# paulmillr/noble-bls12-381

Measured on AMD Instinct MI355X. Metric: pairings/sec, higher is better.
Workload: dtype int64; 1 GPU; batch of 4096 independent BLS12-381 pairings per GPU (Miller loop + final exponentiation, inputs pre-validated, bit-exact vs reference), inputs/outputs resident in HBM; batch_per_gpu=4096, batches_in_flight=12

## Files before the change

### include/nbls.h

```cpp
#ifndef NBLS_H
#define NBLS_H
#include <stddef.h>
#include <stdint.h>
#ifdef __cplusplus
extern "C" {
#endif

typedef struct nbls_ctx nbls_ctx;

#define NBLS_OK 0
#define NBLS_EINVAL (-1)
#define NBLS_EHIP (-2)
#define NBLS_ENOSUP (-3)
#define NBLS_ENOGPU (-4)
#define NBLS_EDECODE (-5)

int nbls_init(int device_id, nbls_ctx** out);
void nbls_destroy(nbls_ctx* ctx);
const char* nbls_strerror(int code);
int nbls_last_hip_error(nbls_ctx* ctx);

int nbls_pairing_batch(nbls_ctx* ctx, size_t n, const uint8_t* g1_aff, const uint8_t* g2_aff, int with_final_exp, int validate,
                       uint8_t* out_fp12, int8_t* status);
int nbls_pairing_batch_dev(nbls_ctx* ctx, size_t n, const void* d_g1_aff, const void* d_g2_aff, int with_final_exp,
// ... 193 lines not shown
                                            uint8_t* out_proofs48 , int8_t* status );
int  nbls_kzg_recover_cells_and_proofs_fk20(nbls_ctx* ctx, const nbls_kzg_fk20* fk, size_t n, const uint32_t* cell_offsets, const uint32_t* cell_index, const uint8_t* cells,
                                            uint8_t* out_cells, uint8_t* out_proofs48 , int8_t* status );

#define NBLS_ST_G16_C 30
typedef struct nbls_groth16_vk nbls_groth16_vk;
int  nbls_groth16_vk_create(nbls_ctx* ctx, size_t m, const uint8_t* alpha_g1_48, const uint8_t* beta_g2_96, const uint8_t* gamma_g2_96, const uint8_t* delta_g2_96,
                            const uint8_t* ic48 , int8_t* status , nbls_groth16_vk** out);
void nbls_groth16_vk_destroy(nbls_groth16_vk* vk);
int  nbls_groth16_vk_inputs(const nbls_groth16_vk* vk, size_t* m);
int  nbls_groth16_verify(nbls_ctx* ctx, const nbls_groth16_vk* vk, size_t n, const uint8_t* proofs192, const uint8_t* inputs32 , const uint8_t* seed32 ,
                         int* all_ok, int8_t* status );
int  nbls_groth16_prepare_inputs(nbls_ctx* ctx, const nbls_groth16_vk* vk, size_t n, const uint8_t* inputs32, uint8_t* out48 , int8_t* status );
int  nbls_groth16_input_sums(nbls_ctx* ctx, size_t n, size_t m, const uint8_t* inputs32, const uint8_t* weights32 , const int8_t* pre ,
                             uint8_t* out32 , int8_t* status );

#define NBLS_ST_G16_UNSATISFIED 24
typedef struct {
  unsigned log2_n; size_t n_vars, n_public , n_constraints ;
  const uint32_t *a_rows, *a_cols; const uint8_t* a_vals32;
  const uint32_t *b_rows, *b_cols; const uint8_t* b_vals32;
  const uint32_t *c_rows, *c_cols; const uint8_t* c_vals32;
  const uint8_t *alpha_g1_48, *beta_g1_48, *beta_g2_96, *delta_g1_48, *delta_g2_96;
  const uint8_t *a_query48 , *b_g1_query48 , *b_g2_query96 , *l_query48 , *h_query48 ;
} nbls_groth16_pk_desc;
typedef struct nbls_groth16_pk nbls_groth16_pk;
int  nbls_groth16_pk_create(nbls_ctx* ctx, const nbls_groth16_pk_desc* desc, int8_t* status , nbls_groth16_pk** out);
void nbls_groth16_pk_destroy(nbls_groth16_pk* pk);
int  nbls_groth16_pk_params(const nbls_groth16_pk* pk, unsigned* log2_n, size_t* n_vars, size_t* n_public);
int  nbls_groth16_pk_wiped(nbls_ctx* ctx, nbls_groth16_pk* pk, int* wiped);
int  nbls_groth16_prove(nbls_ctx* ctx, nbls_groth16_pk* pk, size_t n, const uint8_t* witness32 ,
                        const uint8_t* rs32 , uint8_t* out_proofs192, int8_t* status );
int  nbls_groth16_quotient(nbls_ctx* ctx, unsigned log2_n, size_t n, const uint8_t* a32, const uint8_t* b32, const uint8_t* c32 ,
                           uint8_t* out_h32 , int8_t* status );

int nbls_verify_batch_partial_dev(nbls_ctx* ctx, size_t n, const void* d_sig96 , const void* d_uniform256, const void* d_pk48,
                                  void* d_out_fp12, int* zero_flag, int8_t* pk_status , void* stream);

int nbls_miller_product_partial(nbls_ctx* ctx, size_t n, const uint8_t* g1_aff, const uint8_t* g2_aff, int validate, void** d_partial, int8_t* status);
int nbls_verify_batch_partial(nbls_ctx* ctx, size_t n, const uint8_t* sig96 , const uint8_t* msgs, const uint32_t* offsets, const uint8_t* pk48,
                              const uint8_t* dst, size_t dst_len, void** d_partial, int* zero_flag, int8_t* pk_status );
int nbls_miller_product_partial_into(nbls_ctx* ctx, size_t n, const uint8_t* g1_aff, const uint8_t* g2_aff, int validate, void* d_dst576, int8_t* status);
int nbls_verify_batch_partial_into(nbls_ctx* ctx, size_t n, const uint8_t* sig96 , const uint8_t* msgs, const uint32_t* offsets, const uint8_t* pk48,
                                   const uint8_t* dst, size_t dst_len, void* d_dst576, int* zero_flag, int8_t* pk_status );
const char* nbls_config_describe(void);
#define NBLS_ABI_VERSION 5
int nbls_abi_version(void);
int nbls_context_device(nbls_ctx* ctx);

int nbls_hw_queues(int* set_by_library);
typedef struct nbls_pool nbls_pool;
int nbls_pool_init(int device_id, int depth , nbls_pool** out);
#define NBLS_POOL_SPREAD_PRIORITIES 1u
int nbls_pool_init_ex(int device_id, int depth , unsigned flags, nbls_pool** out);
int nbls_pool_stream_priority(nbls_pool* p, int i, int* priority);
void nbls_pool_destroy(nbls_pool* p);
int nbls_pool_depth(const nbls_pool* p);
nbls_ctx* nbls_pool_context(nbls_pool* p, int i);
int nbls_pool_next_slot(nbls_pool* p);
int nbls_pool_pairing_batch_dev(nbls_pool* p, size_t n, const void* d_g1, const void* d_g2, int with_final_exp, void* d_out, int* slot);
int nbls_pool_synchronize(nbls_pool* p);

typedef struct nbls_multi nbls_multi;
int nbls_init_multi(int n_devices, const int* device_ids, nbls_multi** out);
void nbls_destroy_multi(nbls_multi* m);
int nbls_multi_device_count(const nbls_multi* m);
nbls_ctx* nbls_multi_context(nbls_multi* m, int i);
int nbls_multi_peer_access(const nbls_multi* m, int i);
int nbls_multi_pairing_batch(nbls_multi* m, size_t n, const uint8_t* g1_aff, const uint8_t* g2_aff, int with_final_exp, int validate,
                             uint8_t* out_fp12, int8_t* status);
int nbls_multi_miller_product(nbls_multi* m, size_t n, const uint8_t* g1_aff, const uint8_t* g2_aff, int final_exp, int validate,
                              uint8_t* out_fp12, int8_t* status);
int nbls_multi_verify_batch(nbls_multi* m, size_t n, const uint8_t* sig96, const uint8_t* msgs, const uint32_t* offsets, const uint8_t* pk48,
                            const uint8_t* dst, size_t dst_len, int* ok);

int nbls_program_stats(nbls_ctx* ctx, int prog, uint32_t* out8);
int nbls_device_synchronize(nbls_ctx* ctx);
int nbls_placement_probe(nbls_ctx* ctx, size_t n, uint64_t* out_blocks);
int nbls_field_kernel_raw(nbls_ctx* ctx, int kind, int form, size_t n, const uint8_t* in_raw, uint8_t* out_raw);
#define NBLS_N_PROGRAMS 128
#define NBLS_TUNE_SPLIT_MILLER_MIN 1
#define NBLS_TUNE_HALVES_MIN 2
#define NBLS_TUNE_EXPC_MIN 3
#define NBLS_TUNE_CHAIN_MAX 4
#define NBLS_TUNE_VERIFY_CHUNKS 5
#define NBLS_TUNE_VERIFY_LAST_PCT 6
#define NBLS_TUNE_VERIFY_PIPE_MIN 7
#define NBLS_TUNE_SAC_MAX 8
#define NBLS_TUNE_PT_LS2_MAX 9
#define NBLS_TUNE_WIDE_MAX 10
#define NBLS_TUNE_H2C_NORM_MIN 11
#define NBLS_TUNE_INV_WIDE_MAX 12
#define NBLS_TUNE_LS_MAX 13
#define NBLS_TUNE_LS2_MAX 14
#define NBLS_TUNE_POLY_SLAB 15
#define NBLS_TUNE_MSMB_WINDOW 16
#define NBLS_TUNE_MSMB_BIG 17
#define NBLS_TUNE_MSMB_SLAB 18
#define NBLS_TUNE_CELLS_CHUNK 20
#define NBLS_TUNE_G16_CHUNK 22
#define NBLS_TUNE_FE_TAIL_CHAIN 24
#define NBLS_TUNE_NTT_TAIL_BITS 26
#define NBLS_TUNE_NTT_PASS_BITS 27
#define NBLS_TUNE_FE_HEAD_CHAIN 29
#define NBLS_TUNE_INV_PRIO 30
#define NBLS_TUNE_G16P_ROW_WAVE 31
int nbls_set_tuning(nbls_ctx* ctx, int key, long long value);
int nbls_program_count(void);
// ... 14 lines not shown
```

### noble-bls12-381_amd/csrc/nbls_internal.h

```cpp
#pragma once
#include <hip/hip_runtime.h>
#include "config.h"
#include <cstdio>
#include <cstring>
#include <mutex>
#include <vector>
#include <initializer_list>
#include <new>
#include "nbls.h"
#include "programs.h"
#include "consts_gen.h"
#include "fp_inv.h"
#include "pow_exec.h"
#include "sha256.h"
#include "curve.h"
#include "bufs.h"
#include "verifier_frame.h"
#include <thread>

#include "launchers.h"
#include "wide_exec.h"
#include "aot.h"
#include <map>
#include <tuple>
// ... 189 lines not shown
    if (ctx->ev_last && ctx->ev_last_set && ctx->last_stream != s) hipStreamWaitEvent(s, ctx->ev_last, 0);
  }
  ~StreamOrder() { if (ctx->ev_last && hipEventRecord(ctx->ev_last, s) == hipSuccess) { ctx->ev_last_set = true; ctx->last_stream = s; } }
};

struct ForkGuard {
  bool armed = true; void* keys = nullptr; size_t key_bytes = 0;
  ~ForkGuard() { if (armed) { (void)hipDeviceSynchronize(); if (keys) (void)hipMemset(keys, 0, key_bytes); } }
};
struct Window {
  size_t first = 0;
  int half = 0;
  bool beside = false;
};
struct HostIO {
  nbls_ctx* ctx; std::vector<size_t> mine; hipStream_t s = nullptr; std::vector<std::pair<void*, size_t>> secrets; bool wiped = false;
  ~HostIO() {
    if (!mine.empty()) (void)hipStreamSynchronize(s ? s : ctx->stream);
    if (!wiped) for (auto& k : secrets) (void)hipMemset(k.first, 0, k.second);
    for (size_t i : mine) ctx->io_pool[i].busy = false;
  }
  void secret(void* p, size_t n) { if (p && n) secrets.push_back({p, n}); }
  int wipe(hipStream_t st) { for (auto& k : secrets) if (hipMemsetAsync(k.first, 0, k.second, st) != hipSuccess) return NBLS_EHIP; wiped = true; return NBLS_OK; }
  void* alloc(size_t n) {
    if (!n) n = 1;
    auto& pool = ctx->io_pool;
    size_t best = (size_t)-1;
    for (size_t i = 0; i < pool.size(); i++)
      if (!pool[i].busy && pool[i].p && pool[i].cap >= n && pool[i].cap / 4 <= n && (best == (size_t)-1 || pool[i].cap < pool[best].cap)) best = i;
    if (best != (size_t)-1) { pool[best].busy = true; mine.push_back(best); return pool[best].p; }
    static const size_t cap_bytes = (size_t)env_long("NBLS_IO_POOL_MB", 1024) << 20;
    const size_t cap = n + n / 8 + 256;
    for (size_t i = 0; i < pool.size() && ctx->io_pool_bytes + cap > cap_bytes; i++)
      if (!pool[i].busy && pool[i].p) { hipFree(pool[i].p); ctx->io_pool_bytes -= pool[i].cap; pool[i].p = nullptr; pool[i].cap = 0; }
    void* p = nullptr;
    if (hipMalloc(&p, cap) != hipSuccess) { (void)hipGetLastError(); return nullptr; }
    ctx->io_pool_bytes += cap;
    size_t slot = (size_t)-1;
    for (size_t i = 0; i < pool.size(); i++) if (!pool[i].p) { slot = i; break; }
    if (slot == (size_t)-1) { pool.push_back({nullptr, 0, false}); slot = pool.size() - 1; }
    pool[slot] = {p, cap, true};
    mine.push_back(slot);
    return p;
  }
};
#define LOCKED(ctx) std::lock_guard<std::recursive_mutex> g_((ctx)->mu); HIPCHK(hipSetDevice((ctx)->device)); hipStream_t s = (ctx)->stream; StreamOrder order_((ctx), s)
static inline hipStream_t call_stream(nbls_ctx* ctx, void* stream) { return stream ? (hipStream_t)stream : ctx->stream; }
#define DEV_ENTER(ctx, stream) std::lock_guard<std::recursive_mutex> g_((ctx)->mu); HIPCHK(hipSetDevice((ctx)->device)); hipStream_t s = call_stream((ctx), (stream)); StreamOrder order_((ctx), s)
#define WHOLE_CALL(ctx) std::lock_guard<std::recursive_mutex> whole_call_((ctx) ? (ctx)->mu : g_null_mu)

struct VerifyIn;
int nbls_init_prio(int device_id, int prio, nbls_ctx** out);
int nbls_stream_priority(nbls_ctx* ctx, int* prio);
bool checked_mode();
bool aot_enabled();
int upload_program(nbls_ctx* ctx, DevProgram& d, const Program& p, const int k);
int upload(nbls_ctx* ctx, ProgId id);
int upload_extra(nbls_ctx* ctx, ExtraProg id);
void free_program(DevProgram& d);
bool wide_applies(const nbls_ctx* ctx, const DevProgram& d, int id, size_t n);
hipEvent_t timing_event(nbls_ctx* ctx);
void aot_seg(AotSeg& g, const DevProgram& d, const IOBuf* bufs);
void kernel_args(KernelArgs& ka, const nbls_ctx* ctx, const DevProgram& d, size_t n);
int run_dev(nbls_ctx* ctx, const DevProgram& d, int id, size_t n, const BufList& bufs, hipStream_t s, const uint32_t* n_dev, const uint32_t* item_index);
int run(nbls_ctx* ctx, ProgId id, size_t n, const BufList& bufs, hipStream_t s, const uint32_t* n_dev = nullptr, const uint32_t* item_index = nullptr);
int run_inv(nbls_ctx* ctx, size_t n, const void* in, void* out, hipStream_t s);
bool chains_enabled();
int run_chain(nbls_ctx* ctx, size_t n, const ChainLink* links, size_t count, hipStream_t s);
int ensure_scratch(nbls_ctx* ctx, size_t n);
int ensure_expc_scratch(nbls_ctx* ctx);
int ensure_io(nbls_ctx* ctx, size_t n);
int ensure_lines(nbls_ctx* ctx, size_t n);
int need(nbls_ctx* ctx, Slot i, size_t bytes, uint8_t** out);
int ensure_fork_event(nbls_ctx* ctx);
int ensure_side(nbls_ctx* ctx);
int ensure_side2(nbls_ctx* ctx);
int ensure_half_stream(nbls_ctx* ctx);
int ensure_pinned(nbls_ctx* ctx, size_t bytes);
int ensure_pinned_out(nbls_ctx* ctx, size_t bytes);
size_t pow_wide_max();
int run_pow(nbls_ctx* ctx, int which, size_t n, const void* in, void* out, hipStream_t s, uint8_t* scratch = nullptr);
int run_inv_buf(nbls_ctx* ctx, size_t n, const void* in, void* out, hipStream_t s);
ProgId ls_variant(nbls_ctx* ctx, ProgId id, size_t n);
ProgId pt_ls2_variant(nbls_ctx* ctx, ProgId id, size_t n);
int reduce_product(nbls_ctx* ctx, size_t n, uint8_t** result, hipStream_t s);
int expx(nbls_ctx* ctx, const Window& w, size_t n, uint8_t* in, uint8_t* out, hipStream_t s);
int final_exp_pipeline(nbls_ctx* ctx, const Window& w, size_t n, uint8_t* f_raw, void* d_out, hipStream_t s);
int finish_single(nbls_ctx* ctx, const Window& w, uint8_t* f_raw, int final_exp, void* d_out, hipStream_t s);
int pairing_core(nbls_ctx* ctx, const Window& w, size_t n, const void* d_g1, const void* d_g2, int with_final_exp, void* d_out, hipStream_t s, bool two_programs);
int lines_acc(nbls_ctx* ctx, size_t c, const uint8_t* g1, const uint8_t* g2, uint8_t* L, size_t GR, uint8_t* acc_out, size_t h, hipStream_t s);
int miller_values(nbls_ctx* ctx, size_t n, const void* d_g1, const void* d_g2, size_t* m_out, hipStream_t s);
int acc_prepared(nbls_ctx* ctx, size_t n, const void* d_g1, const void* d_tables, size_t table_stride, hipStream_t s);
int partial_buffer(nbls_ctx* ctx, void* d_dst, uint8_t** dst);
int miller_product_partial_core(nbls_ctx* ctx, size_t n, const uint8_t* g1, const uint8_t* g2, int validate, void* d_dst, void** d_partial, int8_t* status);
int dev_validate(nbls_ctx* ctx, bool g2, size_t n, const void* d_pts, void* d_status, hipStream_t s);
int dev_decompress(nbls_ctx* ctx, bool g2, size_t n, const void* d_in, void* d_out, void* d_status, hipStream_t s, const DecSlots& sl = DEC_MAIN, int mode = 0, size_t io = 0,
    size_t ntot = 0);
int dev_clear_g2(nbls_ctx* ctx, size_t n, void* in, uint8_t* base, uint8_t* S, void* out, void* N, hipStream_t s);
int dev_hash_to_g2(nbls_ctx* ctx, size_t n, const void* d_uniform, void* d_out, hipStream_t s, size_t io = 0, size_t ntot = 0, uint8_t** proj = nullptr);
int to_affine(nbls_ctx* ctx, bool g2, size_t n, const void* Pj, void* N, void* NI, void* d_out, void* d_status, hipStream_t s, bool norm = true);
int dev_point_sum(nbls_ctx* ctx, bool g2, size_t n, const void* d_pts, void* d_out, void* d_status, hipStream_t s);
int decompress_host(nbls_ctx* ctx, bool g2, size_t n, const uint8_t* in, uint8_t* out, int8_t* status);
int dev_expand(nbls_ctx* ctx, size_t n, const uint8_t* msgs, const uint32_t* offs, const uint8_t* dst, size_t dst_len, uint8_t** d_uniform, hipStream_t s, unsigned len_in_bytes = 256);
int sum_host(nbls_ctx* ctx, bool g2, size_t n, const uint8_t* pts, uint8_t* out, int8_t* status);
int dev_hash_to_g1(nbls_ctx* ctx, int count, size_t n, const void* d_uniform, void* d_out, hipStream_t s);
int dev_encode_to_g2(nbls_ctx* ctx, size_t n, const void* d_uniform, void* d_out, hipStream_t s);
// ... 105 lines not shown
```

### noble-bls12-381_amd/csrc/nbls_multi.cpp

```cpp
#include <hip/hip_runtime.h>
#include <condition_variable>
#include <cstdio>
#include <cstdlib>
#include <cstring>
#include <deque>
#include <functional>
#include <mutex>
#include <thread>
#include <vector>
#include "nbls.h"
#include "config.h"
#include "pool_levels.h"

#define EXPORT extern "C" __attribute__((visibility("default")))

struct GatherLanes;
struct CallBuffers {
  std::vector<uint8_t*> part;
  uint8_t* gather = nullptr;
  GatherLanes* lanes = nullptr;
};
struct Worker {
  std::thread th; std::mutex mu; std::condition_variable cv; std::deque<std::function<void()>> q; bool stop = false;
  void run() {
    for (;;) {
      std::function<void()> f;
      { std::unique_lock<std::mutex> l(mu); cv.wait(l, [&] { return stop || !q.empty(); }); if (q.empty()) return; f = std::move(q.front()); q.pop_front(); }
      f();
    }
  }
  void post(std::function<void()> f) { { std::lock_guard<std::mutex> l(mu); q.push_back(std::move(f)); } cv.notify_one(); }
  void start() { th = std::thread([this] { run(); }); }
  void finish() { { std::lock_guard<std::mutex> l(mu); stop = true; } cv.notify_one(); if (th.joinable()) th.join(); }
};
struct nbls_multi {
  std::vector<Worker*> workers;
  std::vector<nbls_ctx*> ctx;
  std::vector<int> dev;
  std::vector<int> peer;
  std::mutex mu;
  std::vector<CallBuffers*> free_sets;
  std::vector<CallBuffers*> all_sets;
};
struct GatherLanes { std::vector<hipStream_t> s; std::vector<hipEvent_t> e; hipStream_t fin = nullptr; };

static void free_set(nbls_multi* m, CallBuffers* b) {
  for (size_t g = 0; g < b->part.size(); g++) if (b->part[g]) { hipSetDevice(m->dev[g]); hipFree(b->part[g]); }
  hipSetDevice(m->dev[0]);
  if (b->gather) hipFree(b->gather);
  if (b->lanes) {
    for (hipStream_t st : b->lanes->s) if (st) hipStreamDestroy(st);
    for (hipEvent_t e : b->lanes->e) if (e) hipEventDestroy(e);
    if (b->lanes->fin) hipStreamDestroy(b->lanes->fin);
    delete b->lanes;
  }
  delete b;
}
static CallBuffers* take_set(nbls_multi* m) {
  {
    std::lock_guard<std::mutex> g(m->mu);
    if (!m->free_sets.empty()) { CallBuffers* b = m->free_sets.back(); m->free_sets.pop_back(); return b; }
  }
  int prev = 0; hipGetDevice(&prev);
  CallBuffers* b = new CallBuffers();
  b->part.assign(m->dev.size(), nullptr);
// ... 107 lines not shown
EXPORT int nbls_multi_miller_product(nbls_multi* m, size_t n, const uint8_t* g1, const uint8_t* g2, int final_exp, int validate, uint8_t* out, int8_t* status) {
  if (!m || m->ctx.empty() || !out || (n && (!g1 || !g2))) return NBLS_EINVAL;
  const size_t G = m->ctx.size();
  SetLease lease(m);
  if (!lease.b) return NBLS_EHIP;
  CallBuffers* b = lease.b;
  int r = on_every_device(m, G, [&](size_t g) {
    size_t lo, hi; shard(n, G, g, &lo, &hi);
    void* p = b->part[g];
    return nbls_miller_product_partial_into(m->ctx[g], hi - lo, g1 + lo * 96, g2 + lo * 192, validate, p, status ? status + lo : nullptr);
  });
  if (r) { if (r == NBLS_EDECODE) memset(out, 0, 576); return r; }
  return finish(m, b, G, final_exp, out);
}

EXPORT int nbls_multi_verify_batch(nbls_multi* m, size_t n, const uint8_t* sig96, const uint8_t* msgs, const uint32_t* offsets, const uint8_t* pk48,
                                   const uint8_t* dst, size_t dst_len, int* ok) {
  if (!m || m->ctx.empty() || !ok || !n || !sig96 || !offsets || !pk48 || !dst) return NBLS_EINVAL;
  size_t G = m->ctx.size();
  if (G > n) G = n;
  SetLease lease(m);
  if (!lease.b) return NBLS_EHIP;
  CallBuffers* b = lease.b;
  std::vector<int> zero(G, 0);
  int r = on_every_device(m, G, [&](size_t g) {
    size_t lo, hi; shard(n, G, g, &lo, &hi);
    void* p = b->part[g];
    return nbls_verify_batch_partial_into(m->ctx[g], hi - lo, g == 0 ? sig96 : nullptr, msgs, offsets + lo, pk48 + lo * 48, dst, dst_len, p, &zero[g], nullptr);
  });
  if (r) return r;
  for (int z : zero) if (z) { *ok = 0; return NBLS_OK; }
  uint8_t e[576];
  r = finish(m, b, G, 1, e);
  if (r) return r;
  bool one = e[47] == 1; for (int i = 0; i < 576 && one; i++) if (i != 47 && e[i]) one = false;
  *ok = one ? 1 : 0;
  return NBLS_OK;
}

static const unsigned POOL_FE_TAIL_CHAIN = 3;
static const unsigned POOL_FE_HEAD_CHAIN = 1, POOL_INV_PRIO = 1;
static int g_queues_set_by_library = 0;
__attribute__((constructor)) static void nbls_on_load() {
  if (getenv("NBLS_KEEP_HW_QUEUES")) return;
  if (!getenv("GPU_MAX_HW_QUEUES")) { setenv("GPU_MAX_HW_QUEUES", "22", 0); g_queues_set_by_library = 1; }
}
EXPORT int nbls_hw_queues(int* set_by_library) {
  if (set_by_library) *set_by_library = g_queues_set_by_library;
  const char* v = getenv("GPU_MAX_HW_QUEUES");
  return v && *v ? atoi(v) : 0;
}
int nbls_init_prio(int device_id, int prio, nbls_ctx** out);
int nbls_stream_priority(nbls_ctx* ctx, int* prio);
static const int POOL_SPREAD_LEVELS = 3;
struct nbls_pool { std::vector<nbls_ctx*> ctx; std::mutex mu; size_t next = 0; int device = 0; };
EXPORT void nbls_pool_destroy(nbls_pool* p) { if (!p) return; for (nbls_ctx* c : p->ctx) nbls_destroy(c); delete p; }
EXPORT int nbls_pool_init(int device_id, int depth, nbls_pool** out) { return nbls_pool_init_ex(device_id, depth, 0, out); }
EXPORT int nbls_pool_init_ex(int device_id, int depth, unsigned flags, nbls_pool** out) {
  if (!out || depth < 1 || depth > 64 || (flags & ~NBLS_POOL_SPREAD_PRIORITIES)) return NBLS_EINVAL;
  const int q = nbls_hw_queues(nullptr), eff = q > 0 ? q : 4;
  std::vector<int> levels(1, 0);
  const long spread_env = nbls::env_long("NBLS_POOL_SPREAD", -1);
  if ((spread_env < 0 ? (flags & NBLS_POOL_SPREAD_PRIORITIES) != 0 : spread_env != 0) && depth > eff) {
    int least = 0, greatest = 0;
    if (hipSetDevice(device_id) != hipSuccess) return NBLS_ENOGPU;
    if (hipDeviceGetStreamPriorityRange(&least, &greatest) != hipSuccess) return NBLS_EHIP;
    levels = nbls::pool_priority_levels(greatest, least, (int)nbls::env_long("NBLS_POOL_SPREAD_LEVELS", POOL_SPREAD_LEVELS));
    if (levels.size() == 1) levels[0] = 0;
  }
  {
    static bool warned = false;
    if (depth > eff * (int)levels.size() && !warned) {
      warned = true;
      fprintf(stderr, "nbls: pool of %d contexts on %d hardware queues (GPU_MAX_HW_QUEUES %s): streams will share queues and their kernels serialise; "
                      "set GPU_MAX_HW_QUEUES >= depth (<= 22) before the first HIP call of the process\n",
              depth, eff, q > 0 ? "as set" : "unset");
    }
  }
  nbls_pool* p = new nbls_pool(); p->device = device_id;
  for (int i = 0; i < depth; i++) {
    nbls_ctx* c = nullptr;
    const int r = nbls_init_prio(device_id, levels[(size_t)nbls::pool_priority_level(i, depth, eff, (int)levels.size())], &c);
    if (r) { nbls_pool_destroy(p); return r; }
    p->ctx.push_back(c);
    if (depth > 1) {
      nbls_set_tuning(c, NBLS_TUNE_SPLIT_MILLER_MIN, 0);
      if (nbls::env_long("NBLS_PIPELINE_CHAIN", 0) != 1) nbls_set_tuning(c, NBLS_TUNE_CHAIN_MAX, 0);
      nbls_set_tuning(c, NBLS_TUNE_LS_MAX, 0); nbls_set_tuning(c, NBLS_TUNE_LS2_MAX, 0);
      nbls_set_tuning(c, NBLS_TUNE_FE_TAIL_CHAIN, nbls::fe_tail_chain_default(POOL_FE_TAIL_CHAIN));
      nbls_set_tuning(c, NBLS_TUNE_FE_HEAD_CHAIN, nbls::fe_head_chain_default(POOL_FE_HEAD_CHAIN));
      nbls_set_tuning(c, NBLS_TUNE_INV_PRIO, nbls::inv_prio_default(POOL_INV_PRIO));
      nbls_set_tuning(c, NBLS_TUNE_INV_WIDE_MAX, 256);
    }
  }
  *out = p;
  return NBLS_OK;
}
EXPORT int nbls_pool_stream_priority(nbls_pool* p, int i, int* priority) { return p && i >= 0 && i < (int)p->ctx.size() ? nbls_stream_priority(p->ctx[i], priority) : NBLS_EINVAL; }
EXPORT int nbls_pool_depth(const nbls_pool* p) { return p ? (int)p->ctx.size() : 0; }
EXPORT nbls_ctx* nbls_pool_context(nbls_pool* p, int i) { return p && i >= 0 && i < (int)p->ctx.size() ? p->ctx[i] : nullptr; }
EXPORT int nbls_pool_pairing_batch_dev(nbls_pool* p, size_t n, const void* d_g1, const void* d_g2, int with_final_exp, void* d_out, int* slot) {
  if (!p || p->ctx.empty()) return NBLS_EINVAL;
  size_t k;
  { std::lock_guard<std::mutex> l(p->mu); k = p->next++ % p->ctx.size(); }
  if (slot) *slot = (int)k;
  return nbls_pairing_batch_dev(p->ctx[k], n, d_g1, d_g2, with_final_exp, d_out, nullptr);
}
EXPORT int nbls_pool_next_slot(nbls_pool* p) { if (!p || p->ctx.empty()) return -1; std::lock_guard<std::mutex> l(p->mu); return (int)(p->next % p->ctx.size()); }
EXPORT int nbls_pool_synchronize(nbls_pool* p) { return p && !p->ctx.empty() ? nbls_device_synchronize(p->ctx[0]) : NBLS_EINVAL; }
```

### noble-bls12-381_amd/csrc/runtime.cpp

```cpp
#include "nbls_internal.h"

std::recursive_mutex g_null_mu;
bool checked_mode() {
#if defined(NBLS_CHECKED)
  return true;
#else
  static const bool on = env_long("NBLS_CHECKED", 0) != 0;
  return on;
#endif
}
bool aot_enabled() { static const bool on = env_long("NBLS_AOT", 1) != 0; return on; }
int upload(nbls_ctx* ctx, ProgId id) {
  DevProgram& d = ctx->prog[id];
  if (d.p) return NBLS_OK;
  return upload_program(ctx, d, get_program(id), aot_enabled() ? nbls_aot_index((int)id) : -1);
}
int upload_extra(nbls_ctx* ctx, ExtraProg id) {
  DevProgram& d = ctx->extra[id];
  if (d.p) return NBLS_OK;
  return upload_program(ctx, d, get_extra_program(id), aot_enabled() ? nbls_aot_extra_index((int)id) : -1);
}
void free_program(DevProgram& d) {
  for (void* p : {(void*)d.steps, (void*)d.descs, (void*)d.consts, (void*)d.aot_steps, (void*)d.aot_descs}) if (p) hipFree(p);
  d = DevProgram();
// ... 202 lines not shown
  int r = ensure_fork_event(ctx); if (r) return r;
  if (!ctx->side2 && hipStreamCreateWithFlags(&ctx->side2, hipStreamNonBlocking) != hipSuccess) { ctx->side2 = nullptr; ctx->last_hip = (int)hipGetLastError(); return NBLS_EHIP; }
  if (!ctx->ev_join2 && hipEventCreateWithFlags(&ctx->ev_join2, hipEventDisableTiming) != hipSuccess) { ctx->last_hip = (int)hipGetLastError(); return NBLS_EHIP; }
  return NBLS_OK;
}
int ensure_half_stream(nbls_ctx* ctx) {
  if (!ctx->half_stream && (hipStreamCreateWithFlags(&ctx->half_stream, hipStreamNonBlocking) != hipSuccess || hipEventCreateWithFlags(&ctx->ev_half_fork, hipEventDisableTiming) != hipSuccess ||
                            hipEventCreateWithFlags(&ctx->ev_half_join, hipEventDisableTiming) != hipSuccess)) { ctx->last_hip = (int)hipGetLastError(); return NBLS_EHIP; }
  return NBLS_OK;
}
int ensure_pinned(nbls_ctx* ctx, size_t bytes) {
  if (bytes <= ctx->pinned_cap) return NBLS_OK;
  if (ctx->pinned) { hipHostFree(ctx->pinned); ctx->pinned = nullptr; ctx->pinned_cap = 0; }
  const size_t cap = bytes + bytes / 4 + 4096;
  HIPCHK(hipHostMalloc((void**)&ctx->pinned, cap, hipHostMallocDefault));
  ctx->pinned_cap = cap;
  return NBLS_OK;
}
int ensure_pinned_out(nbls_ctx* ctx, size_t bytes) {
  if (bytes <= ctx->pinned_out_cap) return NBLS_OK;
  if (ctx->pinned_out) { hipHostFree(ctx->pinned_out); ctx->pinned_out = nullptr; ctx->pinned_out_cap = 0; }
  const size_t cap = bytes + bytes / 4 + 4096;
  HIPCHK(hipHostMalloc((void**)&ctx->pinned_out, cap, hipHostMallocDefault));
  ctx->pinned_out_cap = cap;
  return NBLS_OK;
}
int need(nbls_ctx* ctx, Slot i, size_t bytes, uint8_t** out) {
  if (bytes > ctx->sb_cap[i]) {
    if (ctx->sb[i]) hipFree(ctx->sb[i]);
    ctx->sb[i] = nullptr; ctx->sb_cap[i] = 0;
    size_t cap = bytes + bytes / 8 + 4096;
    HIPCHK(hipMalloc(&ctx->sb[i], cap));
    ctx->sb_cap[i] = cap;
  }
  *out = ctx->sb[i];
  return NBLS_OK;
}
size_t pow_wide_max() { static const size_t v = (size_t)env_long("NBLS_POW_WIDE_MAX", 3072); return v; }
int run_pow(nbls_ctx* ctx, int which, size_t n, const void* in, void* out, hipStream_t s, uint8_t* scratch) {
  int is_fp2 = which == 1 || which == 2;
  if (n <= pow_wide_max()) {
    LAUNCHCHK(nbls_pow_wide_launch((unsigned)n, in, out, ctx->nib[which], ctx->nnib[which], which == 1 ? 8 : which == 2 ? 7 : 0, s));
    return NBLS_OK;
  }
  if (!scratch) { int r = need(ctx, SB_POW_TABLE, n * POW_TAB * (is_fp2 ? 2 : 1) * RAW, &scratch); if (r) return r; }
  LAUNCHCHK(nbls_fp_pow_launch((unsigned)n, in, out, ctx->nib[which], ctx->nnib[which], scratch, which == 1 ? 8 : which == 2 ? 7 : 0, s));
  return NBLS_OK;
}

EXPORT int nbls_init(int device_id, nbls_ctx** out) { return nbls_init_prio(device_id, 0, out); }
int nbls_stream_priority(nbls_ctx* ctx, int* prio) {
  if (!ctx || !prio) return NBLS_EINVAL;
  if (hipStreamGetPriority(ctx->stream, prio) != hipSuccess) { ctx->last_hip = (int)hipGetLastError(); return NBLS_EHIP; }
  return NBLS_OK;
}
int nbls_init_prio(int device_id, int prio, nbls_ctx** out) {
  if (!out) return NBLS_EINVAL;
  int count = 0;
  if (hipGetDeviceCount(&count) != hipSuccess || count <= 0) return NBLS_ENOGPU;
  if (device_id < 0 || device_id >= count) return NBLS_EINVAL;
  nbls_ctx* ctx = new nbls_ctx();
  ctx->device = device_id;
  if (hipSetDevice(device_id) != hipSuccess) { delete ctx; return NBLS_ENOGPU; }
  if (hipStreamCreateWithPriority(&ctx->stream, hipStreamDefault, prio) != hipSuccess) { delete ctx; return NBLS_EHIP; }
  if (hipMalloc(&ctx->qp_table, (size_t)QP_TABLE_ENTRIES * RAW_WORDS * 4) != hipSuccess || hipMemcpy(ctx->qp_table, qp_table_words(), (size_t)QP_TABLE_ENTRIES * RAW_WORDS * 4,
      hipMemcpyHostToDevice) != hipSuccess) { delete ctx; return NBLS_EHIP; }
  {
    std::vector<u32> ul((size_t)LINE_ELEMS * RAW_WORDS, 0);
    for (int j = 0; j < N_LINES; j++) memcpy(&ul[(size_t)6 * j * RAW_WORDS], NBLS_R1, NLIMBS * 4);
    if (hipMalloc(&ctx->unit_lines, LINE_BYTES) != hipSuccess || hipMemcpy(ctx->unit_lines, ul.data(), LINE_BYTES, hipMemcpyHostToDevice) != hipSuccess) { delete ctx; return NBLS_EHIP; }
  }
  u32 one[12 * SLOT_WORDS]; memset(one, 0, sizeof one); memcpy(one, NBLS_R1, NLIMBS * 4);
  if (hipMalloc(&ctx->one12, F12) != hipSuccess || hipMemcpy(ctx->one12, one, F12, hipMemcpyHostToDevice) != hipSuccess) { delete ctx; return NBLS_EHIP; }
  {
    const uint64_t* exps[4] = {NBLS_EXP_P_PLUS_1_DIV_4, NBLS_EXP_P2_PLUS_7_DIV_16, NBLS_EXP_P2_MINUS_9_DIV_16, NBLS_EXP_P_MINUS_3_DIV_4};
    const int bits[4] = {NBLS_P_PLUS_1_DIV_4_BITS, NBLS_P2_PLUS_7_DIV_16_BITS, NBLS_P2_MINUS_9_DIV_16_BITS, NBLS_P_MINUS_3_DIV_4_BITS};
    for (int k = 0; k < 4; k++) {
      std::vector<unsigned char> ops;
      if (k == 1 || k == 2) {
        uint64_t K[6]; for (int j = 0; j < 6; j++) K[j] = NBLS_EXP_P_MINUS_3_DIV_4[j];
        K[0] -= 2;
        for (int j = 0; j < 6; j++) K[j] = (K[j] >> 2) | (j < 5 ? K[j + 1] << 62 : 0);
        ops = pow_make_ops(K, 377);
      } else ops = pow_make_ops(exps[k], bits[k]);
      ctx->nnib[k] = (int)(ops.size() / 2);
      if (hipMalloc(&ctx->nib[k], ops.size()) != hipSuccess || hipMemcpy(ctx->nib[k], ops.data(), ops.size(), hipMemcpyHostToDevice) != hipSuccess) { delete ctx; return NBLS_EHIP; }
    }
    uint8_t ng[96];
    auto be = [](uint8_t* o, const u32* limbs) { u32 w[12]; limbs_to_words(w,
        limbs); for (int i = 0; i < 12; i++) { u32 v = w[11 - i]; o[4 * i] = v >> 24; o[4 * i + 1] = v >> 16; o[4 * i + 2] = v >> 8; o[4 * i + 3] = v; } };
    be(ng, NBLS_G1X_RAW); be(ng + 48, NBLS_NEG_G1Y_RAW);
    uint8_t gg[96]; be(gg, NBLS_G1X_RAW); be(gg + 48, NBLS_G1Y_RAW);
    if (hipMalloc(&ctx->gen_g1, 96) != hipSuccess || hipMemcpy(ctx->gen_g1, gg, 96, hipMemcpyHostToDevice) != hipSuccess) { delete ctx; return NBLS_EHIP; }
    u32 id1[3 * SLOT_WORDS] = {0}, id2[6 * SLOT_WORDS] = {0}; memcpy(id1 + SLOT_WORDS, NBLS_R1, NLIMBS * 4); memcpy(id2 + 2 * SLOT_WORDS, NBLS_R1, NLIMBS * 4);
    if (hipMalloc(&ctx->neg_g1, 96) != hipSuccess || hipMemcpy(ctx->neg_g1, ng, 96, hipMemcpyHostToDevice) != hipSuccess ||
        hipMalloc(&ctx->ident_g1, 3 * RAW) != hipSuccess || hipMemcpy(ctx->ident_g1, id1, 3 * RAW, hipMemcpyHostToDevice) != hipSuccess ||
        hipMalloc(&ctx->ident_g2, 6 * RAW) != hipSuccess || hipMemcpy(ctx->ident_g2, id2, 6 * RAW, hipMemcpyHostToDevice) != hipSuccess) { delete ctx; return NBLS_EHIP; }
  }
  for (int i = 0; i < P_COUNT; i++) { if (i == P_G1_MUL || i == P_G2_MUL || i == P_G1_MUL_W3 || i == P_G1_MUL64 || i == P_G2_MUL_W3 || i == P_G1_MUL_FIXED || i == P_G2_MUL_GLS || i == P_G2_MUL_SAC
      || i == P_G2_MUL_SAC_LS2 || i == P_EXPC_SQ || i == P_EXPC_DEC_A || i == P_EXPC_DEC_B || i == P_H2C_B || i == P_H2C_C || i == P_T_SWU || i == P_T_ISO || i == P_T_CLEAR) continue;
    int r = upload(ctx, (ProgId)i); if (r) { int e = ctx->last_hip; (void)e; nbls_destroy(ctx); return r; } }
  *out = ctx;
  return NBLS_OK;
}

EXPORT void nbls_destroy(nbls_ctx* ctx) {
// ... 49 lines not shown
```

### noble-bls12-381_amd/engine.py

```python
import ctypes as C
import os
try:
    import numpy as _np
except ImportError:
    _np = None

_HERE = os.path.dirname(os.path.abspath(__file__))
ABI_VERSION = 5
PROGRAMS = []
DST_DEFAULT = b'BLS_SIG_BLS12381G2_XMD:SHA-256_SSWU_RO_NUL_'


class NblsError(RuntimeError):
    pass


def lib_path():
    return os.environ.get('NBLS_LIBRARY') or os.path.join(_HERE, 'libnbls.so')


class Groth16PkDesc(C.Structure):
    _fields_ = ([('log2_n', C.c_uint), ('n_vars', C.c_size_t), ('n_public', C.c_size_t), ('n_constraints', C.c_size_t)] +
                [(m + f, C.c_void_p) for m in 'abc' for f in ('_rows', '_cols', '_vals32')] +
                [(f, C.c_void_p) for f in ('alpha_g1_48', 'beta_g1_48', 'beta_g2_96', 'delta_g1_48', 'delta_g2_96', 'a_query48', 'b_g1_query48', 'b_g2_query96', 'l_query48', 'h_query48')])
# ... 84 lines not shown
    lib.nbls_kzg_fk20_params.argtypes = [vp, C.POINTER(C.c_uint), C.POINTER(C.c_uint)]
    lib.nbls_kzg_compute_cells_and_proofs_fk20.argtypes = [vp, vp, sz, vp, vp, vp, vp]
    lib.nbls_kzg_recover_cells_and_proofs_fk20.argtypes = [vp, vp, sz, vp, vp, vp, vp, vp, vp]
    lib.nbls_groth16_vk_create.argtypes = [vp, sz, vp, vp, vp, vp, vp, vp, C.POINTER(vp)]
    lib.nbls_groth16_vk_destroy.argtypes = [vp]
    lib.nbls_groth16_vk_destroy.restype = None
    lib.nbls_groth16_vk_inputs.argtypes = [vp, C.POINTER(sz)]
    lib.nbls_groth16_verify.argtypes = [vp, vp, sz, vp, vp, vp, C.POINTER(i32), vp]
    lib.nbls_groth16_prepare_inputs.argtypes = [vp, vp, sz, vp, vp, vp]
    lib.nbls_groth16_input_sums.argtypes = [vp, sz, sz, vp, vp, vp, vp, vp]
    lib.nbls_groth16_pk_create.argtypes = [vp, C.POINTER(Groth16PkDesc), vp, C.POINTER(vp)]
    lib.nbls_groth16_pk_destroy.argtypes = [vp]
    lib.nbls_groth16_pk_destroy.restype = None
    lib.nbls_groth16_pk_params.argtypes = [vp, C.POINTER(C.c_uint), C.POINTER(sz), C.POINTER(sz)]
    lib.nbls_groth16_pk_wiped.argtypes = [vp, vp, C.POINTER(i32)]
    lib.nbls_groth16_prove.argtypes = [vp, vp, sz, vp, vp, vp, vp]
    lib.nbls_groth16_quotient.argtypes = [vp, C.c_uint, sz, vp, vp, vp, vp, vp]
    lib.nbls_keyset_create.argtypes = [vp, sz, vp, vp, C.POINTER(vp)]
    lib.nbls_keyset_destroy.argtypes = [vp]
    lib.nbls_keyset_destroy.restype = None
    lib.nbls_keyset_size.argtypes = [vp, C.POINTER(sz)]
    lib.nbls_verify_batch_dev_inputs.argtypes = [vp, sz, vp, vp, vp, C.POINTER(i32), vp, vp]
    lib.nbls_verify_batch_msgs_dev.argtypes = [vp, sz, vp, vp, vp, vp, vp, sz, C.POINTER(i32), vp]
    lib.nbls_verify_batch_partial_dev.argtypes = [vp, sz, vp, vp, vp, vp, C.POINTER(i32), vp, vp]
    lib.nbls_g2_prepare.argtypes = [vp, sz, vp, vp]
    lib.nbls_g2_prepare_dev.argtypes = [vp, sz, vp, vp, vp]
    lib.nbls_lines_to_wire_dev.argtypes = [vp, sz, vp, vp, vp]
    lib.nbls_lines_from_wire_dev.argtypes = [vp, sz, vp, vp, vp]
    lib.nbls_pairing_prepared_dev.argtypes = [vp, sz, vp, vp, sz, i32, vp, vp]
    lib.nbls_miller_product_prepared_dev.argtypes = [vp, sz, vp, vp, sz, i32, vp, vp]
    lib.nbls_pairing_prepared.argtypes = [vp, sz, vp, vp, sz, i32, i32, vp]
    lib.nbls_set_tuning.argtypes = [vp, i32, C.c_longlong]
    lib.nbls_field_kernel_raw.argtypes = [vp, i32, i32, sz, vp, vp]
    lib.nbls_map_uniform_batch.argtypes = [vp, i32, sz, vp, vp, vp]
    for nm in ('nbls_g1_from_hex_batch', 'nbls_g2_from_hex_batch', 'nbls_g2_from_signature_batch'):
        getattr(lib, nm).argtypes = [vp, sz, vp, sz, vp, vp]
    lib.nbls_g1_to_hex_batch.argtypes = [vp, sz, vp, vp, i32, vp]
    lib.nbls_g2_to_hex_batch.argtypes = [vp, sz, vp, vp, i32, vp]
    lib.nbls_g1_clear_cofactor_batch.argtypes = [vp, sz, vp, vp, vp]
    lib.nbls_g2_clear_cofactor_batch.argtypes = [vp, sz, vp, vp, vp]
    lib.nbls_init_multi.argtypes = [i32, C.POINTER(i32), C.POINTER(vp)]
    lib.nbls_destroy_multi.argtypes = [vp]
    lib.nbls_multi_device_count.argtypes = [vp]
    lib.nbls_multi_peer_access.argtypes = [vp, i32]
    lib.nbls_multi_pairing_batch.argtypes = [vp, sz, vp, vp, i32, i32, vp, vp]
    lib.nbls_multi_miller_product.argtypes = [vp, sz, vp, vp, i32, i32, vp, vp]
    lib.nbls_multi_verify_batch.argtypes = [vp, sz, vp, vp, vp, vp, vp, sz, C.POINTER(i32)]
    lib.nbls_program_name.restype = C.c_char_p
    lib.nbls_program_name.argtypes = [i32]
    lib.nbls_context_device.argtypes = [vp]
    lib.nbls_pool_init.argtypes = [i32, i32, C.POINTER(vp)]
    lib.nbls_pool_init_ex.argtypes = [i32, i32, C.c_uint, C.POINTER(vp)]
    lib.nbls_pool_stream_priority.argtypes = [vp, i32, C.POINTER(i32)]
    lib.nbls_pool_destroy.argtypes = [vp]
    lib.nbls_pool_depth.argtypes = [vp]
    lib.nbls_pool_context.restype = vp
    lib.nbls_pool_context.argtypes = [vp, i32]
    lib.nbls_pool_next_slot.argtypes = [vp]
    lib.nbls_pool_pairing_batch_dev.argtypes = [vp, sz, vp, vp, i32, vp, C.POINTER(i32)]
    lib.nbls_pool_synchronize.argtypes = [vp]
    lib.nbls_program_kernel.restype = C.c_char_p
    lib.nbls_program_kernel.argtypes = [vp, i32]
    lib.nbls_extra_program_kernel.restype = C.c_char_p
    lib.nbls_extra_program_kernel.argtypes = [vp, C.c_char_p]
    if lib.nbls_abi_version() != ABI_VERSION:
        raise NblsError('libnbls.so has ABI %d, this binding is written for ABI %d (rebuild: make -C noble-bls12-381_amd/csrc)' % (lib.nbls_abi_version(), ABI_VERSION))
    if not PROGRAMS:
        PROGRAMS.extend(lib.nbls_program_name(k).decode() for k in range(lib.nbls_program_count()))
    lib.nbls_timing_enable.argtypes = [vp, i32]
    lib.nbls_timing_read.argtypes = [vp, C.POINTER(C.c_float), C.POINTER(C.c_uint32)]
    return lib


def group_messages(msgs):
    seen, distinct, index = {}, [], []
    for m in msgs:
        m = bytes(m)
        g = seen.get(m)
        if g is None:
            g = seen[m] = len(distinct)
            distinct.append(m)
        index.append(g)
    return distinct, index


class _DeviceHandle:
    _destroy = _thing = None

    def __init__(self, lib, handle):
        self.lib = lib
        self.h = handle

    def _get(self, getter, *ctypes_out):
        out = [t(0) for t in ctypes_out]
        if self.h is None or getattr(self.lib, getter)(self.h, *[C.byref(o) for o in out]) != 0:
            raise NblsError('%s: the %s is closed' % (type(self).__name__, self._thing))
        return [o.value for o in out]

    def close(self):
        if getattr(self, 'h', None):
            getattr(self.lib, self._destroy)(self.h)
        self.h = None

    def __del__(self):
        try:
            self.close()
# ... 1068 lines not shown
```

### noble-bls12-381_amd/pipeline.py

```python
import ctypes as C

from .engine import Engine, NblsError, load_library


class PairingPipeline:

    POOL_SPREAD_PRIORITIES = 1

    def __init__(self, device_id=0, depth=12, spread_priorities=True):
        assert depth >= 1
        self.lib = load_library()
        h = C.c_void_p()
        r = self.lib.nbls_pool_init_ex(device_id, depth, self.POOL_SPREAD_PRIORITIES if spread_priorities else 0, C.byref(h))
        if r != 0:
            raise NblsError('nbls_pool_init_ex failed: %s (code %d)' % (self.lib.nbls_strerror(r).decode(), r))
        self.h = h
        self.depth = depth
        self.engines = [Engine(_handle=self.lib.nbls_pool_context(self.h, i)) for i in range(depth)]

    def close(self):
        if getattr(self, 'h', None):
            for e in self.engines:
                e.close()
            self.lib.nbls_pool_destroy(self.h)
            self.h = None

    def __del__(self):
        try:
            self.close()
        except Exception:
            pass

    def stream_priorities(self):
        out = []
        for i in range(self.depth):
            v = C.c_int()
            r = self.lib.nbls_pool_stream_priority(self.h, i, C.byref(v))
            if r != 0:
                raise NblsError('nbls_pool_stream_priority: code %d' % r)
            out.append(v.value)
        return out

    @property
    def slot(self):
        return self.lib.nbls_pool_next_slot(self.h)

    def submit(self, n, d_g1, d_g2, d_out, with_final_exp=True):
        r = self.lib.nbls_pool_pairing_batch_dev(self.h, n, d_g1, d_g2, int(with_final_exp), d_out, None)
        if r != 0:
            raise NblsError('nbls_pool_pairing_batch_dev: %s (code %d)' % (self.lib.nbls_strerror(r).decode(), r))

    def synchronize(self):
        r = self.lib.nbls_pool_synchronize(self.h)
        if r != 0:
            raise NblsError('nbls_pool_synchronize: code %d' % r)
```

Before: 3.065 million pairings/s.

## Balance pool submissions across streams by outstanding-batch count with event rings

Adds a balancing mode to the stream pool that tracks outstanding batches per stream using per-stream rings of HIP events. Each submission goes to the least-loaded stream, capped at a maximum number of in-flight batches per stream, instead of plain round-robin. The aim is to stop work piling up behind slow or low-priority streams so the GPU stays evenly fed. In exchange it adds event records and queries per submit, and the host can sleep-poll when every stream is full, which may throttle submission.

Result: faster. 3.175 million pairings/s (median of 6 runs) (+3.6%).

```diff
diff --git a/include/nbls.h b/include/nbls.h
--- a/include/nbls.h
+++ b/include/nbls.h
@@ -269,8 +269,10 @@
 typedef struct nbls_pool nbls_pool;
 int nbls_pool_init(int device_id, int depth , nbls_pool** out);
 #define NBLS_POOL_SPREAD_PRIORITIES 1u
+#define NBLS_POOL_BALANCE 2u
 int nbls_pool_init_ex(int device_id, int depth , unsigned flags, nbls_pool** out);
 int nbls_pool_stream_priority(nbls_pool* p, int i, int* priority);
+int nbls_pool_outstanding(nbls_pool* p, int i, int* n);
 void nbls_pool_destroy(nbls_pool* p);
 int nbls_pool_depth(const nbls_pool* p);
 nbls_ctx* nbls_pool_context(nbls_pool* p, int i);
diff --git a/noble-bls12-381_amd/csrc/nbls_internal.h b/noble-bls12-381_amd/csrc/nbls_internal.h
--- a/noble-bls12-381_amd/csrc/nbls_internal.h
+++ b/noble-bls12-381_amd/csrc/nbls_internal.h
@@ -265,6 +265,7 @@
 struct VerifyIn;
 int nbls_init_prio(int device_id, int prio, nbls_ctx** out);
 int nbls_stream_priority(nbls_ctx* ctx, int* prio);
+int nbls_record_event(nbls_ctx* ctx, hipEvent_t ev);
 bool checked_mode();
 bool aot_enabled();
 int upload_program(nbls_ctx* ctx, DevProgram& d, const Program& p, const int k);
diff --git a/noble-bls12-381_amd/csrc/nbls_multi.cpp b/noble-bls12-381_amd/csrc/nbls_multi.cpp
--- a/noble-bls12-381_amd/csrc/nbls_multi.cpp
+++ b/noble-bls12-381_amd/csrc/nbls_multi.cpp
@@ -1,4 +1,5 @@
 #include <hip/hip_runtime.h>
+#include <chrono>
 #include <condition_variable>
 #include <cstdio>
 #include <cstdlib>
@@ -11,6 +12,7 @@
 #include "nbls.h"
 #include "config.h"
 #include "pool_levels.h"
+#include "pool_pick.h"
 
 #define EXPORT extern "C" __attribute__((visibility("default")))
 
@@ -224,12 +226,51 @@
 }
 int nbls_init_prio(int device_id, int prio, nbls_ctx** out);
 int nbls_stream_priority(nbls_ctx* ctx, int* prio);
-static const int POOL_SPREAD_LEVELS = 3;
-struct nbls_pool { std::vector<nbls_ctx*> ctx; std::mutex mu; size_t next = 0; int device = 0; };
-EXPORT void nbls_pool_destroy(nbls_pool* p) { if (!p) return; for (nbls_ctx* c : p->ctx) nbls_destroy(c); delete p; }
+int nbls_record_event(nbls_ctx* ctx, hipEvent_t ev);
+static const int POOL_SPREAD_LEVELS = 3, POOL_MAX_OUTSTANDING = 2;
+struct PoolRing { std::vector<hipEvent_t> ev; int head = 0; };
+struct nbls_pool {
+  std::vector<nbls_ctx*> ctx; std::mutex mu; size_t next = 0; int device = 0;
+  bool balance = false; int K = 0;
+  std::vector<PoolRing> ring; std::vector<int> outstanding;
+  int last = -1, latched = -1;
+};
+static int pool_refresh(nbls_pool* p) {
+  for (size_t i = 0; i < p->ring.size(); i++) {
+    PoolRing& r = p->ring[i];
+    while (p->outstanding[i] > 0) {
+      const hipError_t e = hipEventQuery(r.ev[(size_t)r.head]);
+      if (e == hipErrorNotReady) { (void)hipGetLastError(); break; }
+      if (e != hipSuccess) return NBLS_EHIP;
+      r.head = (r.head + 1) % p->K; p->outstanding[i]--;
+    }
+  }
+  return NBLS_OK;
+}
+static int pool_choose(nbls_pool* p, std::unique_lock<std::mutex>& l, int* k) {
+  for (;;) {
+    if (p->latched >= 0) { *k = p->latched; return NBLS_OK; }
+    const int r = pool_refresh(p);
+    if (r) return r;
+    *k = nbls::pool_pick(p->outstanding.data(), (int)p->outstanding.size(), p->K, p->last);
+    if (*k >= 0) return NBLS_OK;
+    l.unlock();
+    std::this_thread::sleep_for(std::chrono::microseconds(50));
+    l.lock();
+  }
+}
+EXPORT void nbls_pool_destroy(nbls_pool* p) {
+  if (!p) return;
+  for (nbls_ctx* c : p->ctx) nbls_destroy(c);
+  for (PoolRing& r : p->ring) for (hipEvent_t e : r.ev) if (e) hipEventDestroy(e);
+  delete p;
+}
 EXPORT int nbls_pool_init(int device_id, int depth, nbls_pool** out) { return nbls_pool_init_ex(device_id, depth, 0, out); }
 EXPORT int nbls_pool_init_ex(int device_id, int depth, unsigned flags, nbls_pool** out) {
-  if (!out || depth < 1 || depth > 64 || (flags & ~NBLS_POOL_SPREAD_PRIORITIES)) return NBLS_EINVAL;
+  if (!out || depth < 1 || depth > 64 || (flags & ~(NBLS_POOL_SPREAD_PRIORITIES | NBLS_POOL_BALANCE))) return NBLS_EINVAL;
+  const long balance_env = nbls::env_long("NBLS_POOL_BALANCE", -1), max_out = nbls::env_long("NBLS_POOL_MAX_OUTSTANDING", POOL_MAX_OUTSTANDING);
+  if (max_out < 1 || max_out > 8) return NBLS_EINVAL;
+  const bool balance = balance_env < 0 ? (flags & NBLS_POOL_BALANCE) != 0 : balance_env != 0;
   const int q = nbls_hw_queues(nullptr), eff = q > 0 ? q : 4;
   std::vector<int> levels(1, 0);
   const long spread_env = nbls::env_long("NBLS_POOL_SPREAD", -1);
@@ -265,6 +306,14 @@
       nbls_set_tuning(c, NBLS_TUNE_INV_WIDE_MAX, 256);
     }
   }
+  if (balance) {
+    p->balance = true; p->K = (int)max_out;
+    p->outstanding.assign((size_t)depth, 0); p->ring.resize((size_t)depth);
+    for (PoolRing& r : p->ring) {
+      r.ev.assign((size_t)p->K, nullptr);
+      for (hipEvent_t& e : r.ev) if (hipEventCreateWithFlags(&e, hipEventDisableTiming) != hipSuccess) { e = nullptr; (void)hipGetLastError(); nbls_pool_destroy(p); return NBLS_EHIP; }
+    }
+  }
   *out = p;
   return NBLS_OK;
 }
@@ -273,10 +322,48 @@
 EXPORT nbls_ctx* nbls_pool_context(nbls_pool* p, int i) { return p && i >= 0 && i < (int)p->ctx.size() ? p->ctx[i] : nullptr; }
 EXPORT int nbls_pool_pairing_batch_dev(nbls_pool* p, size_t n, const void* d_g1, const void* d_g2, int with_final_exp, void* d_out, int* slot) {
   if (!p || p->ctx.empty()) return NBLS_EINVAL;
+  if (p->balance) {
+    std::unique_lock<std::mutex> l(p->mu);
+    int k = -1;
+    int r = pool_choose(p, l, &k);
+    if (r) return r;
+    p->latched = -1; p->last = k;
+    if (slot) *slot = k;
+    r = nbls_pairing_batch_dev(p->ctx[(size_t)k], n, d_g1, d_g2, with_final_exp, d_out, nullptr);
+    if (r) return r;
+    PoolRing& ring = p->ring[(size_t)k];
+    r = nbls_record_event(p->ctx[(size_t)k], ring.ev[(size_t)((ring.head + p->outstanding[(size_t)k]) % p->K)]);
+    if (r) return r;
+    p->outstanding[(size_t)k]++;
+    return NBLS_OK;
+  }
   size_t k;
   { std::lock_guard<std::mutex> l(p->mu); k = p->next++ % p->ctx.size(); }
   if (slot) *slot = (int)k;
   return nbls_pairing_batch_dev(p->ctx[k], n, d_g1, d_g2, with_final_exp, d_out, nullptr);
 }
-EXPORT int nbls_pool_next_slot(nbls_pool* p) { if (!p || p->ctx.empty()) return -1; std::lock_guard<std::mutex> l(p->mu); return (int)(p->next % p->ctx.size()); }
-EXPORT int nbls_pool_synchronize(nbls_pool* p) { return p && !p->ctx.empty() ? nbls_device_synchronize(p->ctx[0]) : NBLS_EINVAL; }
+EXPORT int nbls_pool_next_slot(nbls_pool* p) {
+  if (!p || p->ctx.empty()) return -1;
+  std::unique_lock<std::mutex> l(p->mu);
+  if (!p->balance) return (int)(p->next % p->ctx.size());
+  int k = -1;
+  if (pool_choose(p, l, &k)) return -1;
+  p->latched = k;
+  return k;
+}
+EXPORT int nbls_pool_outstanding(nbls_pool* p, int i, int* n) {
+  if (!p || !n || i < 0 || i >= (int)p->ctx.size()) return NBLS_EINVAL;
+  if (!p->balance) { *n = 0; return NBLS_OK; }
+  std::lock_guard<std::mutex> l(p->mu);
+  const int r = pool_refresh(p);
+  if (r) return r;
+  *n = p->outstanding[(size_t)i];
+  return NBLS_OK;
+}
+EXPORT int nbls_pool_synchronize(nbls_pool* p) {
+  if (!p || p->ctx.empty()) return NBLS_EINVAL;
+  const int r = nbls_device_synchronize(p->ctx[0]);
+  if (r || !p->balance) return r;
+  std::lock_guard<std::mutex> l(p->mu);
+  return pool_refresh(p);
+}
diff --git a/noble-bls12-381_amd/csrc/pool_pick.h b/noble-bls12-381_amd/csrc/pool_pick.h
--- /dev/null
+++ b/noble-bls12-381_amd/csrc/pool_pick.h
@@ -0,0 +1,12 @@
+#pragma once
+namespace nbls {
+inline int pool_pick(const int* outstanding, int depth, int K, int after) {
+  if (!outstanding || depth < 1 || K < 1) return -1;
+  int start = (after % depth + depth + 1) % depth, best = -1;
+  for (int j = 0; j < depth; j++) {
+    const int i = (start + j) % depth;
+    if (outstanding[i] < K && (best < 0 || outstanding[i] < outstanding[best])) best = i;
+  }
+  return best;
+}
+}
diff --git a/noble-bls12-381_amd/csrc/runtime.cpp b/noble-bls12-381_amd/csrc/runtime.cpp
--- a/noble-bls12-381_amd/csrc/runtime.cpp
+++ b/noble-bls12-381_amd/csrc/runtime.cpp
@@ -278,6 +278,13 @@
 int nbls_stream_priority(nbls_ctx* ctx, int* prio) {
   if (!ctx || !prio) return NBLS_EINVAL;
   if (hipStreamGetPriority(ctx->stream, prio) != hipSuccess) { ctx->last_hip = (int)hipGetLastError(); return NBLS_EHIP; }
+  return NBLS_OK;
+}
+int nbls_record_event(nbls_ctx* ctx, hipEvent_t ev) {
+  if (!ctx || !ev) return NBLS_EINVAL;
+  std::lock_guard<std::recursive_mutex> g_(ctx->mu);
+  HIPCHK(hipSetDevice(ctx->device));
+  HIPCHK(hipEventRecord(ev, ctx->stream));
   return NBLS_OK;
 }
 int nbls_init_prio(int device_id, int prio, nbls_ctx** out) {
diff --git a/noble-bls12-381_amd/engine.py b/noble-bls12-381_amd/engine.py
--- a/noble-bls12-381_amd/engine.py
+++ b/noble-bls12-381_amd/engine.py
@@ -160,6 +160,7 @@
     lib.nbls_pool_init.argtypes = [i32, i32, C.POINTER(vp)]
     lib.nbls_pool_init_ex.argtypes = [i32, i32, C.c_uint, C.POINTER(vp)]
     lib.nbls_pool_stream_priority.argtypes = [vp, i32, C.POINTER(i32)]
+    lib.nbls_pool_outstanding.argtypes = [vp, i32, C.POINTER(i32)]
     lib.nbls_pool_destroy.argtypes = [vp]
     lib.nbls_pool_depth.argtypes = [vp]
     lib.nbls_pool_context.restype = vp
diff --git a/noble-bls12-381_amd/pipeline.py b/noble-bls12-381_amd/pipeline.py
--- a/noble-bls12-381_amd/pipeline.py
+++ b/noble-bls12-381_amd/pipeline.py
@@ -6,12 +6,13 @@
 class PairingPipeline:
 
     POOL_SPREAD_PRIORITIES = 1
+    POOL_BALANCE = 2
 
-    def __init__(self, device_id=0, depth=12, spread_priorities=True):
+    def __init__(self, device_id=0, depth=12, spread_priorities=True, balance=True):
         assert depth >= 1
         self.lib = load_library()
         h = C.c_void_p()
-        r = self.lib.nbls_pool_init_ex(device_id, depth, self.POOL_SPREAD_PRIORITIES if spread_priorities else 0, C.byref(h))
+        r = self.lib.nbls_pool_init_ex(device_id, depth, (self.POOL_SPREAD_PRIORITIES if spread_priorities else 0) | (self.POOL_BALANCE if balance else 0), C.byref(h))
         if r != 0:
             raise NblsError('nbls_pool_init_ex failed: %s (code %d)' % (self.lib.nbls_strerror(r).decode(), r))
         self.h = h
```
